# facebookresearch/gtn

Measured on AMD Instinct MI355X. Metric: CTC forward+backward losses/sec (T=1000, C=256), higher is better.
Workload: dtype f32; 1 GPU; BASELINE config C3: compose(ctc_target, emissions)+forwardScore CTC loss fwd+bwd, T=1000, C=256, U=100, batch=512 per GPU; global_batch=512, parallelism=dp1 (utterance sharding, all_gather of losses), rccl_ranks=0

## Files before the change

### gtn_amd/_capi.py

```python
import ctypes as C
import os

c_graph = C.c_void_p
c_graph_p = C.POINTER(C.c_void_p)
c_i32_p = C.POINTER(C.c_int)
c_i64_p = C.POINTER(C.c_int64)
c_u8_p = C.POINTER(C.c_uint8)
c_f32_p = C.POINTER(C.c_float)

GRAD_FN = C.CFUNCTYPE(C.c_int, C.c_void_p, c_graph_p, C.c_int, c_graph)
CTX_FREE = C.CFUNCTYPE(None, C.c_void_p)

OK, INVALID_ARGUMENT, LOGIC_ERROR, RUNTIME_ERROR, OUT_OF_RANGE, DEVICE_ERROR = range(6)

_SIGS = {
    "gtnx_set_device": [C.c_int],
    "gtnx_get_device": [c_i32_p],
    "gtnx_set_stream": [C.c_void_p],
    "gtnx_compose_mode": [C.c_int, C.POINTER(C.c_int)],
    "gtnx_synchronize": [],
    "gtnx_memory_stats": [C.POINTER(C.c_uint64), C.POINTER(C.c_uint64)],
    "gtnx_empty_cache": [],
    "gtnx_reclaim": [],
    "gtnx_graph_create": [C.c_int, c_graph_p],
# ... 94 lines not shown
    "gtnx_batch_align_stats": [c_i64_p, c_i64_p],
    "gtnx_batch_viterbi_decode": [c_graph, c_graph, C.c_void_p, C.c_void_p, C.c_int64, C.c_void_p, C.c_void_p,
                                  C.c_void_p],
    "gtnx_batch_decode_stats": [c_i64_p, c_i64_p],
    "gtnx_batch_full_connect_stats": [c_i64_p, c_i64_p],
    "gtnx_batch_linear_decode": [c_graph, C.c_void_p, C.c_int, C.c_void_p, C.c_int64, C.c_void_p, C.c_void_p,
                                 C.c_void_p, C.c_void_p],
    "gtnx_batch_linear_decode_stats": [c_i64_p, c_i64_p],
    "gtnx_batch_ctc_beam_decode": [c_graph, C.c_void_p, C.c_int, C.c_int, C.c_int, C.c_int, C.c_void_p, C.c_int64,
                                   C.c_void_p, C.c_void_p],
    "gtnx_batch_ctc_beam_stats": [c_i64_p, c_i64_p],
    "gtnx_batch_linear_shape": [c_graph, c_i32_p, c_i32_p],
    "gtnx_batch_edit_distance": [C.c_void_p, C.c_int64, C.c_void_p, C.c_void_p, C.c_int64, C.c_void_p, C.c_int, C.c_int,
                                 C.c_int, C.c_int, C.c_void_p, C.c_void_p],
    "gtnx_batch_edit_distance_stats": [c_i64_p, c_i64_p],
    "gtnx_batch_backward": [c_graph, C.c_int],
    "gtnx_batch_items": [c_graph, C.c_void_p],
    "gtnx_batch_items_device": [c_graph, C.c_void_p],
    "gtnx_batch_grads_bind_device": [c_graph, C.c_void_p, C.c_void_p],
    "gtnx_batch_grads_device": [c_graph, C.c_void_p, C.c_void_p],
    "gtnx_backward": [c_graph, C.c_int],
    "gtnx_backward_with_grad": [c_graph, c_graph, C.c_int],
    "gtnx_backward_n": [c_graph_p, C.c_int, C.c_int],
    "gtnx_equal": [c_graph, c_graph, c_i32_p],
    "gtnx_isomorphic": [c_graph, c_graph, c_i32_p],
    "gtnx_remove": [c_graph, C.c_int, C.c_int, c_graph_p],
    "gtnx_graph_load_buffer": [C.c_void_p, C.c_size_t, c_graph_p],
    "gtnx_parallel_enter": [],
    "gtnx_parallel_leave": [],
    "gtnx_parallel_flush": [],
# ... 55 lines not shown
```

### gtn_amd/criteria/ctc_criterion.h

```cpp
#pragma once

#include <chrono>
#include <cstdint>
#include <stdexcept>
#include <vector>

#include "gtn/gtn.h"

namespace gtn {
namespace criteria {

inline Graph ctcTargetGraph(const std::vector<int>& target, int blank = 0, bool calcGrad = true) {
  const int L = 2 * (int)target.size() + 1;
  std::vector<uint8_t> st(L, 0), ac(L, 0);
  std::vector<int> src, dst, lab;
  src.reserve(3 * L);
  dst.reserve(3 * L);
  lab.reserve(3 * L);
  for (int l = 0; l < L; l++) {
    const int idx = (l - 1) / 2;
    st[l] = l == 0;
    ac[l] = l == L - 1 || l + 2 == L;
    const int label = l % 2 ? target[idx] : blank;
    src.push_back(l), dst.push_back(l), lab.push_back(label);
// ... 18 lines not shown
    int B,
    int T,
    int C,
    int blank,
    void* lossDev,
    void* gradDev,
    bool targetGrad = true,
    CtcStepTimes* times = nullptr,
    Batch* targetsOut = nullptr,
    const int* frames = nullptr) {
  auto now = [] { return std::chrono::steady_clock::now(); };
  auto ms = [](auto a, auto b) { return std::chrono::duration<double, std::milli>(b - a).count(); };
  if (frames)
    for (int b = 0; b < B; ++b)
      if (frames[b] < 1 || frames[b] > T) throw std::invalid_argument("[ctcLossBatch] a frame count outside 1 .. T");
  auto t0 = now();
  Batch ctcs = Batch::ctcTargets(labels, lengths, B, blank, targetGrad);
  auto t1 = now();
  Batch ems = Batch::linear(B, T, C, emissions, gradDev != nullptr, true, frames);
  std::vector<int64_t> off(B);
  for (int b = 0; b < B; ++b) off[b] = (int64_t)b * T * C;
  if (gradDev) ems.bindGrads(gradDev, off.data());
  auto t2 = now();
  Batch comp = batched::intersect(ctcs, ems);
  auto t3 = now();
  Batch score = batched::forwardScore(comp);
  Batch norm = batched::forwardScore(ems);
  Batch losses = batched::subtract(norm, score, lossDev);
  auto t4 = now();
  if (gradDev) batched::backward(losses);
// ... 81 lines not shown
```

### gtn_amd/csrc/band.hip

```cpp
#include <hip/hip_runtime.h>

#include <algorithm>
#include <cstdlib>
#include <stdexcept>
#include <type_traits>

#include "kernels.h"

#ifdef GTNX_BAND_TIMING
__device__ long long g_band_timing[256];
#endif

namespace gtnx {
namespace {

constexpr float NEGF = -1.0e30f;
constexpr float DEADF = -1.0e29f;
constexpr float LOG2E = 1.44269504088896340736f;
constexpr double LN2 = 0.693147180559945309417;
constexpr int BW = 256;
constexpr int WG = 512;
constexpr int WGB = 768;
constexpr int NBE = 5;
constexpr int NBG = 7;
// ... 317 lines not shown
#define GTNX_BAND_PAIR one
#include "band_forward_body.inc"
#undef GTNX_BAND_PAIR
}

__device__ __forceinline__ BandPair band_patched(BandPair P, const BandPatch& pt) {
  if (pt.on) {
    const int b = P.bidx;
    P.delta = pt.delta + b;
    P.delta_norm = pt.delta_norm ? pt.delta_norm + b : nullptr;
    P.rowlse = pt.rowlse ? pt.rowlse + int64_t(b) * pt.M : nullptr;
    P.norm = nullptr;
    P.em_copy = nullptr;
    P.grad_em = pt.grad_em ? pt.grad_em + int64_t(b) * pt.A : nullptr;
    P.grad_fixed = pt.grad_fixed ? pt.grad_fixed + P.goff : nullptr;
  }
  return P;
}
template <int NPL, bool UNIT, bool GRADG, int K, bool VEC, bool BIG>
__global__ __launch_bounds__(WGB, BIG ? 3 : 6) void band_backward_kernel(const BandPair* __restrict__ pairs, int NSmax, BandPatch patch) {
#define GTNX_BAND_PAIR band_patched(pairs[blockIdx.x], patch)
#include "band_backward_body.inc"
#undef GTNX_BAND_PAIR
}
template <int NPL, bool UNIT, bool GRADG, int K, bool VEC, bool BIG>
__global__ __launch_bounds__(WGB, BIG ? 3 : 6) void band_backward_one_kernel(BandPair one, int NSmax) {
#define GTNX_BAND_PAIR one
#include "band_backward_body.inc"
#undef GTNX_BAND_PAIR
}


__global__ __launch_bounds__(512) void ctc_targets_kernel(const CtcTargetArgs* __restrict__ args, int blank) {
  const CtcTargetArgs a = args[blockIdx.x];
  __shared__ __attribute__((aligned(16))) int tl[256 + 4];
  __shared__ __attribute__((aligned(16))) int tk[256 + 4];
  const int N = a.N, U = (N - 1) >> 1, m = threadIdx.x;
  if (m < 260) {
    const int v = m < U ? a.labels[m] : 0x7fffffff;
    tl[m] = v;
    tk[m] = (m > 0 && m < U && v != a.labels[m - 1]) ? 1 : 0;
  }
  __syncthreads();
  if (m >= N) return;
  const bool odd = (m & 1) != 0;
  const int my = odd ? tl[(m - 1) >> 1] : blank;
  const int skip = odd ? tk[(m - 1) >> 1] : 0;
  const int mi = (m - 1) >> 1;
  const int before = odd ? mi : (m >> 1);
  int rank = 0, skips = 0;
  for (int o = 0; o < U; o += 4) {
    const gtnx_i4 l4 = *reinterpret_cast<const gtnx_i4*>(tl + o), k4 = *reinterpret_cast<const gtnx_i4*>(tk + o);
    const int lo[4] = {l4.x, l4.y, l4.z, l4.w}, ko[4] = {k4.x, k4.y, k4.z, k4.w};
#pragma unroll
    for (int k = 0; k < 4; ++k) {
      const bool front = o + k < before;
      rank += (lo[k] < my || (lo[k] == my && front)) ? 1 : 0;
      skips += front ? ko[k] : 0;
    }
  }
  rank += blank < my ? U + 1 : (blank == my ? (m + 1) >> 1 : 0);
  const int base = (m > 0 ? 2 * m - 1 : 0) + skips;
  GTNX_G BandNode* nd = const_cast<GTNX_G BandNode*>(a.nodes);
  nd[m].lab = my;
  nd[m].aid[0] = base;
  nd[m].aid[1] = m > 0 ? base + 1 : -1;
  nd[m].aid[2] = skip ? base + 2 : -1;
  a.nflags[m] = uint8_t((m == 0 ? NF_START : 0) | (m + 2 >= N ? NF_ACCEPT : 0));
  a.snode[rank] = m;
  a.slab[rank] = my;
  if (m == N - 1 && a.n_arcs) a.n_arcs[0] = base + 1 + (m > 0 ? 1 : 0) + skip;
}

__global__ __launch_bounds__(512) void band_viterbi_kernel(const BandDecode* __restrict__ pairs) {
  const BandDecode P = pairs[blockIdx.x];
  const int T = P.T, C = P.C, N = P.N, NS = P.NS;
  extern __shared__ float lds[];
  const float NINF = -__builtin_inff();
  float* a0 = lds;
  float* a1 = lds + 516;
  float* stage = lds + 1032;
  const int m = threadIdx.x;
  const GTNX_G gtnx_i4* nodes = reinterpret_cast<const GTNX_G gtnx_i4*>(P.nodes);
  int lab = 0;
  float wi[3] = {NINF, NINF, NINF};
  bool accept = false, start = false;
// ... 555 lines not shown
  hipLaunchKernelGGL(band_viterbi_kernel, dim3(n), dim3(512), 4 * size_t(1032 + stage_floats) + 64, st, d_pairs);
}

void launch_asg_fal_targets(const AsgFalArgs* d_args, int n, int n_labels, hipStream_t st) {
  if (n > 0) hipLaunchKernelGGL(asg_fal_targets_kernel, dim3(n), dim3(512), 0, st, d_args, n_labels);
}
void launch_asg_fal_scatter(const float* g, const int* maps, const int64_t* tab, int n_seq, int64_t longest, float* trans_grad,
                            hipStream_t st) {
  if (n_seq > 0 && longest > 0)
    hipLaunchKernelGGL(asg_fal_scatter_kernel, dim3(unsigned(std::min<int64_t>((longest + 255) / 256, 64)), unsigned(n_seq)),
                       dim3(256), 0, st, g, maps, tab, trans_grad);
}
void launch_ctc_targets(const CtcTargetArgs* d_args, int n, int blank, hipStream_t st) {
  if (n > 0) hipLaunchKernelGGL(ctc_targets_kernel, dim3(n), dim3(512), 0, st, d_args, blank);
}

}
```

### gtn_amd/csrc/band_backward_body.inc

```
  constexpr int RNk = K >= 4 ? 4 : K;
  constexpr int NP = K / RNk;
  const BandPair P = GTNX_BAND_PAIR;
  const int T = P.T, C = P.C, NS = P.NS;
  extern __shared__ float lds[];
  const BandLds L = band_lds(C, K, NSmax, true);
  float* ering = lds + L.o_ering;
  float* aring = lds + L.o_aring;
  float* oring = lds + L.o_oring;
  int* snode = reinterpret_cast<int*>(lds + L.o_snode);
  const BandMisc M = band_misc<K>(lds, L);
  float* lser = M.lsep;
  const int CS = L.CS;
  const int wv = __builtin_amdgcn_readfirstlane(threadIdx.x >> 6);
  const bool sweeper = wv < 4;
  const int l = threadIdx.x & 63;
  const int nblocks = (T + K - 1) / K;
  const int nticks = nblocks + 5;
  const GTNX_G double* ao = P.aoff;
  const double z2 = uniform(ao[0]);
  const bool dead = !(z2 > double(DEADF));
  const float ds = uniform(P.delta[0]);
  const bool want_em = P.grad_em != nullptr;
  GTNX_TM_INIT(128);
  constexpr bool SPLIT = !BIG && K >= 2 && GTNX_BWD_SPLIT;
  const float dn_k = P.delta_norm ? uniform(P.delta_norm[0]) : 0.0f;
  float* const rnorm_k = lser + NBG * K;
  auto rows_of_k = [&](int c) { return c < nblocks ? min(K, T - c * K) : 0; };
  auto ring_start = [](int c, int M) { return ((c % M) + M) % M; };
  static_assert((NBGE & (NBGE - 1)) == 0, "the emission ring's position is a mask");
  auto ge_of = [](int c) { return int(unsigned(c) & unsigned(NBGE - 1)); };
  auto ring_step = [](int& v, int M) { v = v + 1 == M ? 0 : v + 1; };
  struct RowSumRegs {
    float in[NPL];
    gtnx_f4 hot[NPL];
  };
  auto rowsum_init = [&](RowSumRegs& R) {
#pragma unroll
    for (int q = 0; q < NPL; ++q) {
      const int mb = 256 * q + 4 * l;
      R.in[q] = mb < NSmax ? 1.0f : 0.0f;
// ... 688 lines not shown
```

### gtn_amd/csrc/band_forward_body.inc

```
#ifndef GTNX_FWD_SHIFT_ROWS
#define GTNX_FWD_SHIFT_ROWS 4
#endif
  constexpr int RNk = K >= GTNX_FWD_SHIFT_ROWS ? GTNX_FWD_SHIFT_ROWS : (K >= 4 ? 4 : K);
  constexpr int NP = K / RNk;
  constexpr int D = 8 / K > GTNX_FWD_DEPTH ? 8 / K : GTNX_FWD_DEPTH;
  const BandPair P = GTNX_BAND_PAIR;
  const int T = P.T, C = P.C, NS = P.NS;
  extern __shared__ float lds[];
  const BandLds L = band_lds(C, K, NSmax, false);
  float* ering = lds + L.o_ering;
  const BandMisc M = band_misc<K>(lds, L);
  const int CS = L.CS;
  const int wv = __builtin_amdgcn_readfirstlane(threadIdx.x >> 6);
  const bool sweeper = wv < 4;
  const int l = threadIdx.x & 63;
  const int nblocks = (T + K - 1) / K;
  const int nticks = nblocks + 3;
  GTNX_TM_INIT(0);

  if (sweeper) {
    __builtin_amdgcn_s_setprio(1);
    const int w = wv;
    const int m0 = threadIdx.x * NPL;
    NodeRegs<NPL> g;
// ... 317 lines not shown
    }
    if (hid < 16) M.red[hid] = normacc;
  }
  GTNX_TM_DUMP();
  lds_barrier();
  if (threadIdx.x == 0) {
    double Mx = double(NEGF);
    for (int k = 0; k < 4; ++k)
      if (M.fin[2 * k] > DEADF) Mx = fmax(Mx, M.find[k] + double(M.fin[2 * k]));
    const bool dead = !(Mx > double(DEADF));
    float S = 0.0f;
    for (int k = 0; k < 4; ++k)
      if (M.fin[2 * k] > DEADF) S += M.fin[2 * k + 1] * ex2(float(M.find[k] + double(M.fin[2 * k]) - Mx));
    const double z2 = dead ? double(NEGF) : Mx + double(lg2(S));
    P.aoff[0] = z2;
    P.score[0] = dead ? -__builtin_inff() : float(z2 * LN2);
    if (P.norm) {
      double n2 = 0.0;
      for (int k = 0; k < 16; ++k) n2 += M.red[k];
      P.norm[0] = n2 < double(DEADF) ? -__builtin_inff() : float(n2 * LN2);
    }
  }
```

### gtn_amd/csrc/batch.cpp

```cpp
#include "batch.h"

#include <algorithm>
#include <atomic>
#include <cstdlib>
#include <cstring>
#include <limits>
#include <unordered_map>
#include <unordered_set>

namespace gtnx {

namespace {

std::atomic<uint64_t> g_batch_seq{1};

struct CompMode {
  int old;
  CompMode() : old(compose_mode_hint(2)) {}
  ~CompMode() { compose_mode_hint(old); }
};

BatchP make_batch(Batch::Kind k, int n, bool cg) {
  auto b = std::make_shared<Batch>();
  b->kind = k;
// ... 369 lines not shown
    st[size_t(l)] = l == 0;
    ac[size_t(l)] = l == L - 1 || l + 2 == L;
    const int label = l % 2 ? t[idx] : blank;
    src.push_back(l), dst.push_back(l), lab.push_back(label);
    if (l > 0) src.push_back(l - 1), dst.push_back(l), lab.push_back(label);
    if (l % 2 && l > 1 && label != t[idx - 1]) src.push_back(l - 2), dst.push_back(l), lab.push_back(label);
  }
  Graph g(cg);
  g.add_nodes(L, st.data(), ac.data());
  g.add_arcs(int(src.size()), src.data(), dst.data(), lab.data(), lab.data(), nullptr);
  g.arc_sort(false);
  return g;
}
}

BatchP batch_ctc_targets(const int* labels, const int* lengths, int n, int blank, bool calc_grad) {
  GTNX_HOST_T("batch.ctc_targets");
  if (n < 0) throw_invalid("[gtnx_batch_ctc_targets] negative batch size");
  BatchP b = make_batch(Batch::CTC_TARGETS, n, calc_grad);
  b->blank = blank;
  b->lab_off.resize(size_t(n) + 1);
  b->lab_off[0] = 0;
  for (int i = 0; i < n; ++i) {
    if (lengths[i] < 0) throw_invalid("[gtnx_batch_ctc_targets] negative length");
    b->lab_off[size_t(i) + 1] = b->lab_off[size_t(i)] + lengths[i];
    b->max_nodes = std::max(b->max_nodes, 2 * lengths[i] + 1);
  }
  const size_t total = size_t(b->lab_off[size_t(n)]);
  b->labels.assign(labels, labels + total);
  int mn = blank;
  b->max_label = blank;
  for (size_t i = 0; i < total; ++i) {
    b->max_label = std::max(b->max_label, labels[i]);
    mn = std::min(mn, labels[i]);
  }
  if (mn < 0 || b->max_nodes > band_max_nodes() || n == 0) {
    std::vector<Graph> gs;
    gs.reserve(size_t(n));
    for (int i = 0; i < n; ++i)
      gs.push_back(ctc_target_graph_host(labels + b->lab_off[size_t(i)], lengths[i], blank, calc_grad));
    return batch_from_graphs(std::move(gs));
  }
  Runtime& rt = Runtime::get();
  const size_t lab_bytes = align_up(sizeof(int) * (total ? total : 1), 256);
  const size_t arg_bytes = align_up(sizeof(CtcTargetArgs) * size_t(n), 256);
  size_t bytes = lab_bytes + arg_bytes;
  b->rec_off.resize(size_t(n));
  for (int i = 0; i < n; ++i) {
    const size_t N = size_t(2 * lengths[i] + 1);
    b->rec_off[size_t(i)] = bytes;
    bytes += align_up(sizeof(BandNode) * N, 64) + align_up(N, 64) + 2 * align_up(4 * N, 64) + 64;
  }
  b->rec_mem = rt.alloc(bytes);
  PinnedMemP pin = rt.alloc_pinned(lab_bytes + arg_bytes);
  std::memcpy(pin->ptr, labels, sizeof(int) * total);
  CtcTargetArgs* args = reinterpret_cast<CtcTargetArgs*>(static_cast<char*>(pin->ptr) + lab_bytes);
  for (int i = 0; i < n; ++i) {
    const size_t N = size_t(2 * lengths[i] + 1);
    char* base = b->rec_mem->as<char>(b->rec_off[size_t(i)]);
    CtcTargetArgs& a = args[size_t(i)];
    a.labels = b->rec_mem->as<int>() + b->lab_off[size_t(i)];
    a.nodes = reinterpret_cast<BandNode*>(base);
    base += align_up(sizeof(BandNode) * N, 64);
    a.nflags = reinterpret_cast<uint8_t*>(base);
    base += align_up(N, 64);
    a.snode = reinterpret_cast<int*>(base);
    base += align_up(4 * N, 64);
    a.slab = reinterpret_cast<int*>(base);
    base += align_up(4 * N, 64);
    a.n_arcs = reinterpret_cast<int*>(base);
    a.N = int(N);
    a.pad = 0;
  }
  rt.h2d_pinned(b->rec_mem->ptr, pin->ptr, lab_bytes + arg_bytes);
  launch_ctc_targets(reinterpret_cast<const CtcTargetArgs*>(b->rec_mem->as<char>(lab_bytes)), n, blank, rt.stream());
  return b;
}


BatchP batch_asg_force_align(const int* labels, const int* lengths, int n, Graph& transitions, int n_labels) {
  if (n < 0) throw_invalid("[gtnx_batch_asg_force_align] negative batch size");
  if (transitions.num_nodes() != int64_t(n_labels) + 1 || transitions.num_arcs() != int64_t(n_labels) * (n_labels + 1))
    throw_invalid("[gtnx_batch_asg_force_align] the transitions graph must have the asgTransitions(N) layout");
  BatchP b = make_batch(Batch::CTC_TARGETS, n, transitions.calc_grad());
  b->fal = true;
  b->trans = transitions;
  b->trans_labels = n_labels;
  b->lab_off.resize(size_t(n) + 1);
  b->lab_off[0] = 0;
  int max_u = 0;
  for (int i = 0; i < n; ++i) {
// ... 1423 lines not shown
```

### gtn_amd/csrc/batch.h

```cpp
#pragma once

#include <memory>
#include <vector>

#include "ops.h"

namespace gtnx {

struct Batch;
using BatchP = std::shared_ptr<Batch>;

struct BatchOp {
  uint64_t seq = 0;
  std::vector<BatchP> inputs;
  virtual void backward(Batch& out) = 0;
  virtual ~BatchOp() {}
};

struct Batch {
  enum Kind { GRAPHS, CTC_TARGETS, LINEAR, PRODUCT, SCALAR };
  Kind kind = GRAPHS;
  int n = 0;
  bool calc_grad = false;

// ... 41 lines not shown
  std::shared_ptr<BatchOp> op;
  bool tape_cleared = false;
  DevMemP g_mem;
  float* g_dev = nullptr;
  std::vector<int64_t> g_off;
  DevMemP dest_mem;
  float* dest = nullptr;

  int64_t elem_size(int b) const;
  ~Batch();
};

BatchP batch_from_graphs(std::vector<Graph> gs);
BatchP batch_ctc_targets(const int* labels, const int* lengths, int n, int blank, bool calc_grad);
BatchP batch_asg_force_align(const int* labels, const int* lengths, int n, Graph& transitions, int n_labels);
BatchP batch_linear(int n, int M, int C, bool calc_grad, const void* dev, bool borrow, const int* rows = nullptr);
BatchP batch_compose(const BatchP& a, const BatchP& b, bool intersect);
BatchP batch_shortest_distance(const BatchP& x, bool tropical);
void batch_full_connect_stats(int64_t* fast, int64_t* fallback);
BatchP batch_viterbi_path(const BatchP& x);
void batch_viterbi_align(const BatchP& x, const int* frames, int* labels_dev, int64_t row_stride, int* tokens_dev,
                         float* scores_dev);
void batch_align_stats(int64_t* fast, int64_t* fallback);
void batch_viterbi_decode(const BatchP& ems, Graph& transitions, const int* frames, int* labels_dev, int64_t row_stride,
                          float* scores_dev, int* collapsed_dev, int* lengths_dev);
void batch_decode_stats(int64_t* fast, int64_t* fallback);
void batch_linear_decode(const BatchP& ems, const int* frames, int blank, int* labels_dev, int64_t row_stride,
                         float* scores_dev, int* collapsed_dev, int* starts_dev, int* lengths_dev);
void batch_linear_decode_stats(int64_t* fast, int64_t* fallback);
void batch_ctc_beam_decode(const BatchP& ems, const int* frames, int blank, int beam, int topn, int nbest,
// ... 21 lines not shown
```

### gtn_amd/csrc/capi.cpp

```cpp
#include <atomic>
#include <chrono>
#include <condition_variable>
#include <cstdlib>
#include <cstring>
#include <mutex>
#include <string>
#include <vector>

#include "batch.h"
#include "ops.h"
#include "ops_internal.h"
#include "region.h"

#define GTNX_API extern "C" __attribute__((visibility("default")))

using namespace gtnx;

namespace {
thread_local std::string g_err;

gtnx_status_t fail(gtnx_status_t s, const std::string& m) {
  g_err = m;
  return s;
}
// ... 730 lines not shown

namespace {
inline BatchP& BH(gtnx_batch_t h) {
  if (!h) throw_invalid("null batch handle");
  return *reinterpret_cast<BatchP*>(h);
}
inline gtnx_batch_t HB(BatchP b) { return reinterpret_cast<gtnx_batch_t>(new BatchP(std::move(b))); }
}
GTNX_API gtnx_status_t gtnx_batch_from_graphs(const gtnx_graph_t* g, int n, gtnx_batch_t* out) {
  return guard([&] { *out = HB(batch_from_graphs(vec(g, n, true))); });
}
GTNX_API gtnx_status_t gtnx_batch_ctc_targets(const int* labels, const int* lengths, int n, int blank, int cg,
                                              gtnx_batch_t* out) {
  return guard([&] { *out = HB(batch_ctc_targets(labels, lengths, n, blank, cg != 0)); });
}
GTNX_API gtnx_status_t gtnx_batch_asg_force_align(const int* labels, const int* lengths, int n, gtnx_graph_t transitions,
                                                  int n_labels, gtnx_batch_t* out) {
  return guard([&] { *out = HB(batch_asg_force_align(labels, lengths, n, G(transitions), n_labels)); });
}
GTNX_API gtnx_status_t gtnx_batch_linear(int n, int M, int N, int cg, const void* dev, int borrow, gtnx_batch_t* out) {
  return guard([&] { *out = HB(batch_linear(n, M, N, cg != 0, dev, borrow != 0)); });
}
GTNX_API gtnx_status_t gtnx_batch_linear_rows(int n, int M, int N, const int* rows, int cg, const void* dev, int borrow,
                                             gtnx_batch_t* out) {
  return guard([&] { *out = HB(batch_linear(n, M, N, cg != 0, dev, borrow != 0, rows)); });
}
GTNX_API gtnx_status_t gtnx_batch_destroy(gtnx_batch_t b) {
  return guard([&] {
    auto* p = reinterpret_cast<BatchP*>(b);
    if (!p) return;
// ... 210 lines not shown
```

### gtn_amd/csrc/kernels.h

```cpp
#pragma once

#include <hip/hip_runtime.h>

#include <cstdint>

#include <atomic>
#include <cstdint>
struct gtnx_first_on_device {
  std::atomic<uint64_t>& done;
  uint64_t bit;
  bool first;
  explicit gtnx_first_on_device(std::atomic<uint64_t>& d) : done(d) {
    int dev = 0;
    (void)hipGetDevice(&dev);
    bit = uint64_t(1) << (dev & 63);
    first = !(done.load(std::memory_order_acquire) & bit);
  }
  gtnx_first_on_device(const gtnx_first_on_device&) = delete;
  ~gtnx_first_on_device() {
    if (first) done.fetch_or(bit, std::memory_order_acq_rel);
  }
  explicit operator bool() const { return first; }
};

// ... 340 lines not shown
  GTNX_G float* alpha;
  GTNX_G double* aoff;
  GTNX_G float* score;
  GTNX_G float* norm;
  GTNX_G float* rowlse;
  const GTNX_G float* delta;
  const GTNX_G float* delta_norm;
  GTNX_G float* grad_em;
  GTNX_G float* grad_fixed;
  int N, T, C, NS;
  int hot;
  int lgrn;
  int n_lab;
  int bidx;
  int64_t goff;
};
struct BandPatch {
  int on;
  int M;
  const GTNX_G float* delta;
  const GTNX_G float* delta_norm;
  GTNX_G float* rowlse;
  GTNX_G float* grad_em;
  GTNX_G float* grad_fixed;
  int64_t A;
};
struct BandDecode {
  const GTNX_G BandNode* nodes;
  const GTNX_G uint8_t* nflags;
  const GTNX_G float* w;
  const GTNX_G float* em;
  GTNX_G uint8_t* bp;
  GTNX_G int* pnode;
  GTNX_G int* path_arc;
  GTNX_G int* path_lab;
  GTNX_G float* path_w;
  GTNX_G int* path_len;
  GTNX_G float* score;
  GTNX_G int* tie;
  const GTNX_G int* rank_in;
// ... 77 lines not shown
void launch_remove_walk(const RemoveArgs& a, bool emit, hipStream_t st);
size_t scan_temp_bytes(int n);
void launch_exclusive_scan(const int* in, int* out, int n, void* temp, size_t temp_bytes, hipStream_t st);
void launch_rational_load(const void* rows, const float* w, const uint8_t* flags, const RationalOut& out, void* temp,
                          hipStream_t st);
struct CtcTargetArgs {
  const GTNX_G int* labels;
  GTNX_G BandNode* nodes;
  GTNX_G uint8_t* nflags;
  GTNX_G int* snode;
  GTNX_G int* slab;
  GTNX_G int* n_arcs;
  int N, pad;
};
void launch_ctc_targets(const CtcTargetArgs* d_args, int n, int blank, hipStream_t st);
struct AsgFalArgs {
  const GTNX_G int* labels;
  const GTNX_G float* trans_w;
  GTNX_G BandNode* nodes;
  GTNX_G uint8_t* nflags;
  GTNX_G int* snode;
  GTNX_G int* slab;
  GTNX_G float* w;
  GTNX_G int* arc_map;
  int U, pad;
};
void launch_asg_fal_targets(const AsgFalArgs* d_args, int n, int n_labels, hipStream_t st);
void launch_asg_fal_scatter(const float* g, const int* maps, const int64_t* tab , int n_seq, int64_t longest,
                            float* trans_grad, hipStream_t st);
int band_max_nodes();
// ... 147 lines not shown
```

### include/gtn/batch.h

```cpp
#pragma once
#include <cstdint>
#include <utility>
#include <vector>

#include "gtn/functions.h"

namespace gtn {

class Batch {
 public:
  Batch() = default;
  explicit Batch(const std::vector<Graph>& graphs) {
    auto h = detail::handles(graphs);
    detail::check(gtnx_batch_from_graphs(h.data(), static_cast<int>(h.size()), &h_));
  }
  Batch(const Batch&) = delete;
  Batch& operator=(const Batch&) = delete;
  Batch(Batch&& o) noexcept : h_(o.h_) { o.h_ = nullptr; }
  Batch& operator=(Batch&& o) noexcept {
    if (this != &o) {
      reset();
      h_ = o.h_;
      o.h_ = nullptr;
    }
// ... 5 lines not shown
    std::vector<int> flat, len;
    len.reserve(targets.size());
    size_t total = 0;
    for (auto& t : targets) total += t.size();
    flat.reserve(total);
    for (auto& t : targets) {
      flat.insert(flat.end(), t.begin(), t.end());
      len.push_back(static_cast<int>(t.size()));
    }
    return ctcTargets(flat.data(), len.data(), static_cast<int>(targets.size()), blank, calcGrad);
  }
  static Batch ctcTargets(const int* labels, const int* lengths, int n, int blank = 0, bool calcGrad = true) {
    Batch b;
    detail::check(gtnx_batch_ctc_targets(labels, lengths, n, blank, calcGrad, &b.h_));
    return b;
  }
  static Batch asgForceAlign(const int* labels, const int* lengths, int n, const Graph& transitions, int numLabels) {
    Batch b;
    detail::check(gtnx_batch_asg_force_align(labels, lengths, n, transitions.handle(), numLabels, &b.h_));
    return b;
  }
  static Batch linear(int n, int M, int N, const void* deviceWeights, bool calcGrad = true, bool borrow = false,
                      const int* rows = nullptr) {
    Batch b;
    if (rows)
      detail::check(gtnx_batch_linear_rows(n, M, N, rows, calcGrad, deviceWeights, borrow, &b.h_));
    else
      detail::check(gtnx_batch_linear(n, M, N, calcGrad, deviceWeights, borrow, &b.h_));
    return b;
  }
// ... 98 lines not shown
```

### include/gtn_amd.h

```cpp
#ifndef GTN_AMD_H
#define GTN_AMD_H

#include <stddef.h>
#include <stdint.h>

#ifdef __cplusplus
extern "C" {
#endif

typedef int gtnx_status_t;
#define GTNX_OK 0
#define GTNX_INVALID_ARGUMENT 1
#define GTNX_LOGIC_ERROR 2
#define GTNX_RUNTIME_ERROR 3
#define GTNX_OUT_OF_RANGE 4
#define GTNX_DEVICE_ERROR 5

typedef struct gtnx_graph_s* gtnx_graph_t;

#define GTNX_EPSILON (-1)

const char* gtnx_last_error(void);
const char* gtnx_version(void);
const char* gtnx_backend(void);
// ... 95 lines not shown
gtnx_status_t gtnx_items_n(const gtnx_graph_t* g, int n, float* out);
gtnx_status_t gtnx_items_device_n(const gtnx_graph_t* g, int n, void* device_out);
gtnx_status_t gtnx_grads_device_n(const gtnx_graph_t* g, int n, void* device_out, const int64_t* offsets);
gtnx_status_t gtnx_grads_bind_device_n(const gtnx_graph_t* g, int n, void* device_out, const int64_t* offsets);

gtnx_status_t gtnx_clone(gtnx_graph_t g, int projection , gtnx_graph_t* out);
gtnx_status_t gtnx_concat(const gtnx_graph_t* g, int n, gtnx_graph_t* out);
gtnx_status_t gtnx_closure(gtnx_graph_t g, gtnx_graph_t* out);
gtnx_status_t gtnx_union(const gtnx_graph_t* g, int n, gtnx_graph_t* out);
gtnx_status_t gtnx_remove(gtnx_graph_t g, int ilabel, int olabel, gtnx_graph_t* out);

typedef struct gtnx_batch_s* gtnx_batch_t;
gtnx_status_t gtnx_batch_from_graphs(const gtnx_graph_t* g, int n, gtnx_batch_t* out);
gtnx_status_t gtnx_batch_ctc_targets(const int* labels, const int* lengths, int n, int blank, int calc_grad,
                                     gtnx_batch_t* out);
gtnx_status_t gtnx_batch_asg_force_align(const int* labels, const int* lengths, int n, gtnx_graph_t transitions,
                                         int n_labels, gtnx_batch_t* out);
gtnx_status_t gtnx_batch_linear(int n, int M, int N, int calc_grad, const void* device_weights, int borrow,
                                gtnx_batch_t* out);
gtnx_status_t gtnx_batch_linear_rows(int n, int M, int N, const int* rows, int calc_grad, const void* device_weights,
                                     int borrow, gtnx_batch_t* out);
gtnx_status_t gtnx_batch_destroy(gtnx_batch_t b);
gtnx_status_t gtnx_batch_size(gtnx_batch_t b, int* out);
gtnx_status_t gtnx_batch_get(gtnx_batch_t b, int i, gtnx_graph_t* out);
gtnx_status_t gtnx_batch_negate(gtnx_batch_t a, gtnx_batch_t* out);
gtnx_status_t gtnx_batch_add(gtnx_batch_t a, gtnx_batch_t b, gtnx_batch_t* out);
gtnx_status_t gtnx_batch_subtract(gtnx_batch_t a, gtnx_batch_t b, gtnx_batch_t* out);
gtnx_status_t gtnx_batch_subtract_into(gtnx_batch_t a, gtnx_batch_t b, void* items_device, gtnx_batch_t* out);
gtnx_status_t gtnx_batch_compose(gtnx_batch_t a, gtnx_batch_t b, gtnx_batch_t* out);
gtnx_status_t gtnx_batch_intersect(gtnx_batch_t a, gtnx_batch_t b, gtnx_batch_t* out);
// ... 61 lines not shown
```

Baseline: 935,700 losses/s.

## Add fused CTC loss path building targets, band forward and backward in few launches

Adds a fused CTC loss route that builds the target records, the band pair table and the arena on the host in one pass. One head kernel both emits the CTC target records and copies the pair table from pinned memory, then runs band forward (writing loss = norm - score directly) and band backward with constant seed deltas. This skips the separate linear batch, intersect, the two forwardScore calls, the subtract and the generic backward dispatch. It costs a large new code path that declines to the old route on unusual shapes, and it reads pinned host memory directly from a kernel.

```diff
diff --git a/gtn_amd/_capi.py b/gtn_amd/_capi.py
--- a/gtn_amd/_capi.py
+++ b/gtn_amd/_capi.py
@@ -132,6 +132,9 @@
     "gtnx_batch_edit_distance": [C.c_void_p, C.c_int64, C.c_void_p, C.c_void_p, C.c_int64, C.c_void_p, C.c_int, C.c_int,
                                  C.c_int, C.c_int, C.c_void_p, C.c_void_p],
     "gtnx_batch_edit_distance_stats": [c_i64_p, c_i64_p],
+    "gtnx_batch_ctc_loss_fused": [C.c_void_p, C.c_void_p, C.c_void_p, C.c_int, C.c_int, C.c_int, C.c_int, C.c_void_p,
+                                  C.c_void_p, C.c_void_p, C.c_int, C.c_void_p, C.POINTER(C.c_int), C.POINTER(C.c_double)],
+    "gtnx_batch_ctc_fused_stats": [c_i64_p, c_i64_p],
     "gtnx_batch_backward": [c_graph, C.c_int],
     "gtnx_batch_items": [c_graph, C.c_void_p],
     "gtnx_batch_items_device": [c_graph, C.c_void_p],
diff --git a/gtn_amd/criteria/ctc_criterion.h b/gtn_amd/criteria/ctc_criterion.h
--- a/gtn_amd/criteria/ctc_criterion.h
+++ b/gtn_amd/criteria/ctc_criterion.h
@@ -56,6 +56,16 @@
   if (frames)
     for (int b = 0; b < B; ++b)
       if (frames[b] < 1 || frames[b] > T) throw std::invalid_argument("[ctcLossBatch] a frame count outside 1 .. T");
+  if (emissions && lengths && lossDev) {
+    Batch fused;
+    double hms[3] = {0, 0, 0};
+    if (Batch::ctcLossFused(emissions, labels, lengths, B, T, C, blank, frames, lossDev, gradDev, targetGrad, &fused, hms) ==
+        GTNX_CTC_FUSED_TAKEN) {
+      if (times) *times = {hms[0], 0, 0, hms[1], hms[2]};
+      if (targetsOut) *targetsOut = std::move(fused);
+      return;
+    }
+  }
   auto t0 = now();
   Batch ctcs = Batch::ctcTargets(labels, lengths, B, blank, targetGrad);
   auto t1 = now();
diff --git a/gtn_amd/csrc/band.hip b/gtn_amd/csrc/band.hip
--- a/gtn_amd/csrc/band.hip
+++ b/gtn_amd/csrc/band.hip
@@ -355,32 +355,44 @@
     P.em_copy = nullptr;
     P.grad_em = pt.grad_em ? pt.grad_em + int64_t(b) * pt.A : nullptr;
     P.grad_fixed = pt.grad_fixed ? pt.grad_fixed + P.goff : nullptr;
+    if (pt.seed) {
+      P.delta = P.score;
+      P.delta_norm = P.score;
+    }
   }
   return P;
 }
 template <int NPL, bool UNIT, bool GRADG, int K, bool VEC, bool BIG>
 __global__ __launch_bounds__(WGB, BIG ? 3 : 6) void band_backward_kernel(const BandPair* __restrict__ pairs, int NSmax, BandPatch patch) {
 #define GTNX_BAND_PAIR band_patched(pairs[blockIdx.x], patch)
+#define GTNX_BAND_DELTA(P) (patch.seed ? patch.seed_delta : uniform((P).delta[0]))
+#define GTNX_BAND_DELTA_NORM(P) (patch.seed ? patch.seed_delta_norm : ((P).delta_norm ? uniform((P).delta_norm[0]) : 0.0f))
 #include "band_backward_body.inc"
+#undef GTNX_BAND_DELTA_NORM
+#undef GTNX_BAND_DELTA
 #undef GTNX_BAND_PAIR
 }
 template <int NPL, bool UNIT, bool GRADG, int K, bool VEC, bool BIG>
 __global__ __launch_bounds__(WGB, BIG ? 3 : 6) void band_backward_one_kernel(BandPair one, int NSmax) {
 #define GTNX_BAND_PAIR one
+#define GTNX_BAND_DELTA(P) uniform((P).delta[0])
+#define GTNX_BAND_DELTA_NORM(P) ((P).delta_norm ? uniform((P).delta_norm[0]) : 0.0f)
 #include "band_backward_body.inc"
+#undef GTNX_BAND_DELTA_NORM
+#undef GTNX_BAND_DELTA
 #undef GTNX_BAND_PAIR
 }
 
 
-__global__ __launch_bounds__(512) void ctc_targets_kernel(const CtcTargetArgs* __restrict__ args, int blank) {
-  const CtcTargetArgs a = args[blockIdx.x];
+__device__ __forceinline__ void ctc_target_records(const CtcTargetArgs& a, const GTNX_G int* src, bool keep, int blank) {
   __shared__ __attribute__((aligned(16))) int tl[256 + 4];
   __shared__ __attribute__((aligned(16))) int tk[256 + 4];
   const int N = a.N, U = (N - 1) >> 1, m = threadIdx.x;
   if (m < 260) {
-    const int v = m < U ? a.labels[m] : 0x7fffffff;
+    const int v = m < U ? src[m] : 0x7fffffff;
     tl[m] = v;
-    tk[m] = (m > 0 && m < U && v != a.labels[m - 1]) ? 1 : 0;
+    tk[m] = (m > 0 && m < U && v != src[m - 1]) ? 1 : 0;
+    if (keep && m < U) const_cast<GTNX_G int*>(a.labels)[m] = v;
   }
   __syncthreads();
   if (m >= N) return;
@@ -411,6 +423,22 @@
   a.snode[rank] = m;
   a.slab[rank] = my;
   if (m == N - 1 && a.n_arcs) a.n_arcs[0] = base + 1 + (m > 0 ? 1 : 0) + skip;
+}
+__global__ __launch_bounds__(512) void ctc_targets_kernel(const CtcTargetArgs* __restrict__ args, int blank) {
+  const CtcTargetArgs a = args[blockIdx.x];
+  ctc_target_records(a, a.labels, false, blank);
+}
+__global__ __launch_bounds__(512) void ctc_head_kernel(const CtcTargetArgs* __restrict__ h_args, int n, int blank,
+                                                       const int* __restrict__ h_labels, const int* d_labels,
+                                                       const gtnx_i4* __restrict__ h_table, gtnx_i4* d_table, int table_vecs) {
+  if (int(blockIdx.x) >= n) {
+    const int stride = int(gridDim.x - n) * 512;
+    for (int i = int(blockIdx.x - n) * 512 + int(threadIdx.x); i < table_vecs; i += stride) d_table[i] = h_table[i];
+    return;
+  }
+  const CtcTargetArgs a = h_args[blockIdx.x];
+  const size_t off = (reinterpret_cast<uintptr_t>(a.labels) - reinterpret_cast<uintptr_t>(d_labels)) / sizeof(int);
+  ctc_target_records(a, (const GTNX_G int*)(h_labels + off), true, blank);
 }
 
 __global__ __launch_bounds__(512) void band_viterbi_kernel(const BandDecode* __restrict__ pairs) {
@@ -996,5 +1024,14 @@
 void launch_ctc_targets(const CtcTargetArgs* d_args, int n, int blank, hipStream_t st) {
   if (n > 0) hipLaunchKernelGGL(ctc_targets_kernel, dim3(n), dim3(512), 0, st, d_args, blank);
 }
-
-}
+void launch_ctc_head(const CtcTargetArgs* h_args, int n, int blank, const int* h_labels, int* d_labels, const void* h_table,
+                     void* d_table, size_t table_bytes, hipStream_t st) {
+  if (n <= 0) return;
+  if (table_bytes % 16 != 0 || table_bytes / 16 > size_t(1) << 30) throw std::logic_error("band.hip: the head's table is copied in 16-byte words");
+  const int vecs = int(table_bytes / 16);
+  const int copiers = std::min((vecs + 511) / 512, 64);
+  hipLaunchKernelGGL(ctc_head_kernel, dim3(n + copiers), dim3(512), 0, st, h_args, n, blank, h_labels, d_labels,
+                     static_cast<const gtnx_i4*>(h_table), static_cast<gtnx_i4*>(d_table), vecs);
+}
+
+}
diff --git a/gtn_amd/csrc/band_backward_body.inc b/gtn_amd/csrc/band_backward_body.inc
--- a/gtn_amd/csrc/band_backward_body.inc
+++ b/gtn_amd/csrc/band_backward_body.inc
@@ -19,11 +19,11 @@
   const GTNX_G double* ao = P.aoff;
   const double z2 = uniform(ao[0]);
   const bool dead = !(z2 > double(DEADF));
-  const float ds = uniform(P.delta[0]);
+  const float ds = GTNX_BAND_DELTA(P);
   const bool want_em = P.grad_em != nullptr;
   GTNX_TM_INIT(128);
   constexpr bool SPLIT = !BIG && K >= 2 && GTNX_BWD_SPLIT;
-  const float dn_k = P.delta_norm ? uniform(P.delta_norm[0]) : 0.0f;
+  const float dn_k = GTNX_BAND_DELTA_NORM(P);
   float* const rnorm_k = lser + NBG * K;
   auto rows_of_k = [&](int c) { return c < nblocks ? min(K, T - c * K) : 0; };
   auto ring_start = [](int c, int M) { return ((c % M) + M) % M; };
diff --git a/gtn_amd/csrc/band_forward_body.inc b/gtn_amd/csrc/band_forward_body.inc
--- a/gtn_amd/csrc/band_forward_body.inc
+++ b/gtn_amd/csrc/band_forward_body.inc
@@ -355,10 +355,14 @@
       if (M.fin[2 * k] > DEADF) S += M.fin[2 * k + 1] * ex2(float(M.find[k] + double(M.fin[2 * k]) - Mx));
     const double z2 = dead ? double(NEGF) : Mx + double(lg2(S));
     P.aoff[0] = z2;
-    P.score[0] = dead ? -__builtin_inff() : float(z2 * LN2);
+    const float sc = dead ? -__builtin_inff() : float(z2 * LN2);
+    P.score[0] = sc;
     if (P.norm) {
       double n2 = 0.0;
       for (int k = 0; k < 16; ++k) n2 += M.red[k];
-      P.norm[0] = n2 < double(DEADF) ? -__builtin_inff() : float(n2 * LN2);
+      const float nrm = n2 < double(DEADF) ? -__builtin_inff() : float(n2 * LN2);
+      P.norm[0] = nrm;
+      GTNX_G float* const loss = (GTNX_BAND_PAIR).loss;
+      if (loss) loss[0] = nrm - sc;
     }
   }
diff --git a/gtn_amd/csrc/batch.cpp b/gtn_amd/csrc/batch.cpp
--- a/gtn_amd/csrc/batch.cpp
+++ b/gtn_amd/csrc/batch.cpp
@@ -2,6 +2,7 @@
 
 #include <algorithm>
 #include <atomic>
+#include <chrono>
 #include <cstdlib>
 #include <cstring>
 #include <limits>
@@ -407,8 +408,8 @@
 }
 }
 
-BatchP batch_ctc_targets(const int* labels, const int* lengths, int n, int blank, bool calc_grad) {
-  GTNX_HOST_T("batch.ctc_targets");
+namespace {
+BatchP ctc_targets_record(const int* labels, const int* lengths, int n, int blank, bool calc_grad, bool* band) {
   if (n < 0) throw_invalid("[gtnx_batch_ctc_targets] negative batch size");
   BatchP b = make_batch(Batch::CTC_TARGETS, n, calc_grad);
   b->blank = blank;
@@ -427,32 +428,33 @@
     b->max_label = std::max(b->max_label, labels[i]);
     mn = std::min(mn, labels[i]);
   }
-  if (mn < 0 || b->max_nodes > band_max_nodes() || n == 0) {
-    std::vector<Graph> gs;
-    gs.reserve(size_t(n));
-    for (int i = 0; i < n; ++i)
-      gs.push_back(ctc_target_graph_host(labels + b->lab_off[size_t(i)], lengths[i], blank, calc_grad));
-    return batch_from_graphs(std::move(gs));
-  }
-  Runtime& rt = Runtime::get();
-  const size_t lab_bytes = align_up(sizeof(int) * (total ? total : 1), 256);
-  const size_t arg_bytes = align_up(sizeof(CtcTargetArgs) * size_t(n), 256);
-  size_t bytes = lab_bytes + arg_bytes;
-  b->rec_off.resize(size_t(n));
+  *band = !(mn < 0 || b->max_nodes > band_max_nodes() || n == 0);
+  return b;
+}
+struct CtcRecLayout {
+  size_t lab_bytes, arg_bytes, bytes;
+};
+CtcRecLayout ctc_targets_layout(Batch& b, const int* lengths) {
+  const int n = b.n;
+  const size_t total = size_t(b.lab_off[size_t(n)]);
+  CtcRecLayout L;
+  L.lab_bytes = align_up(sizeof(int) * (total ? total : 1), 256);
+  L.arg_bytes = align_up(sizeof(CtcTargetArgs) * size_t(n), 256);
+  L.bytes = L.lab_bytes + L.arg_bytes;
+  b.rec_off.resize(size_t(n));
   for (int i = 0; i < n; ++i) {
     const size_t N = size_t(2 * lengths[i] + 1);
-    b->rec_off[size_t(i)] = bytes;
-    bytes += align_up(sizeof(BandNode) * N, 64) + align_up(N, 64) + 2 * align_up(4 * N, 64) + 64;
-  }
-  b->rec_mem = rt.alloc(bytes);
-  PinnedMemP pin = rt.alloc_pinned(lab_bytes + arg_bytes);
-  std::memcpy(pin->ptr, labels, sizeof(int) * total);
-  CtcTargetArgs* args = reinterpret_cast<CtcTargetArgs*>(static_cast<char*>(pin->ptr) + lab_bytes);
-  for (int i = 0; i < n; ++i) {
+    b.rec_off[size_t(i)] = L.bytes;
+    L.bytes += align_up(sizeof(BandNode) * N, 64) + align_up(N, 64) + 2 * align_up(4 * N, 64) + 64;
+  }
+  return L;
+}
+void ctc_targets_args(Batch& b, const int* lengths, CtcTargetArgs* args) {
+  for (int i = 0; i < b.n; ++i) {
     const size_t N = size_t(2 * lengths[i] + 1);
-    char* base = b->rec_mem->as<char>(b->rec_off[size_t(i)]);
+    char* base = b.rec_mem->as<char>(b.rec_off[size_t(i)]);
     CtcTargetArgs& a = args[size_t(i)];
-    a.labels = b->rec_mem->as<int>() + b->lab_off[size_t(i)];
+    a.labels = b.rec_mem->as<int>() + b.lab_off[size_t(i)];
     a.nodes = reinterpret_cast<BandNode*>(base);
     base += align_up(sizeof(BandNode) * N, 64);
     a.nflags = reinterpret_cast<uint8_t*>(base);
@@ -465,9 +467,199 @@
     a.N = int(N);
     a.pad = 0;
   }
-  rt.h2d_pinned(b->rec_mem->ptr, pin->ptr, lab_bytes + arg_bytes);
-  launch_ctc_targets(reinterpret_cast<const CtcTargetArgs*>(b->rec_mem->as<char>(lab_bytes)), n, blank, rt.stream());
+}
+}
+
+BatchP batch_ctc_targets(const int* labels, const int* lengths, int n, int blank, bool calc_grad) {
+  GTNX_HOST_T("batch.ctc_targets");
+  bool band = false;
+  BatchP b = ctc_targets_record(labels, lengths, n, blank, calc_grad, &band);
+  if (!band) {
+    std::vector<Graph> gs;
+    gs.reserve(size_t(n));
+    for (int i = 0; i < n; ++i)
+      gs.push_back(ctc_target_graph_host(labels + b->lab_off[size_t(i)], lengths[i], blank, calc_grad));
+    return batch_from_graphs(std::move(gs));
+  }
+  Runtime& rt = Runtime::get();
+  const size_t total = size_t(b->lab_off[size_t(n)]);
+  const CtcRecLayout L = ctc_targets_layout(*b, lengths);
+  b->rec_mem = rt.alloc(L.bytes);
+  PinnedMemP pin = rt.alloc_pinned(L.lab_bytes + L.arg_bytes);
+  std::memcpy(pin->ptr, labels, sizeof(int) * total);
+  ctc_targets_args(*b, lengths, reinterpret_cast<CtcTargetArgs*>(static_cast<char*>(pin->ptr) + L.lab_bytes));
+  rt.h2d_pinned(b->rec_mem->ptr, pin->ptr, L.lab_bytes + L.arg_bytes);
+  launch_ctc_targets(reinterpret_cast<const CtcTargetArgs*>(b->rec_mem->as<char>(L.lab_bytes)), n, blank, rt.stream());
   return b;
+}
+
+namespace {
+std::atomic<int64_t> g_ctc_fused{0}, g_ctc_declined{0};
+int ctc_declined(int why) {
+  g_ctc_declined.fetch_add(1);
+  return why;
+}
+}
+void batch_ctc_fused_stats(int64_t* fused, int64_t* declined) {
+  if (fused) *fused = g_ctc_fused.load();
+  if (declined) *declined = g_ctc_declined.load();
+}
+int batch_ctc_loss_fused(const void* emissions, const int* labels, const int* lengths, int n, int T, int C, int blank,
+                         const int* frames, void* loss_dev, void* grad_dev, bool target_grad, BatchP* targets_out,
+                         double* host_ms) {
+  GTNX_HOST_T("batch.ctc_loss_fused");
+  if (!emissions || !lengths || !loss_dev) throw_invalid("[gtnx_batch_ctc_loss_fused] null emissions, lengths or loss pointer");
+  if (targets_out) targets_out->reset();
+  if (host_ms) host_ms[0] = host_ms[1] = host_ms[2] = 0.0;
+  const char* sw = std::getenv("GTNX_CTC_FUSED");
+  if (sw && sw[0] == '0') return ctc_declined(CTC_FUSED_OFF);
+  if (std::getenv("GTNX_H2D_KERNEL_BYTES") || std::getenv("GTNX_NO_BAND_PATCH") || std::getenv("GTNX_LAZY_COMPOSE"))
+    return ctc_declined(CTC_FUSED_SWITCH);
+  if (n <= 0 || T < 1 || T > (1 << 20) || C < band_min_labels() || C > band_max_labels()) return ctc_declined(CTC_FUSED_SHAPE);
+  int64_t total_labels = 0;
+  for (int i = 0; i < n; ++i) {
+    if (lengths[i] < 0) return ctc_declined(CTC_FUSED_SHAPE);
+    total_labels += lengths[i];
+  }
+  if (total_labels > 0 && !labels) throw_invalid("[gtnx_batch_ctc_loss_fused] null labels");
+  bool band = false;
+  BatchP fx = ctc_targets_record(labels, lengths, n, blank, target_grad, &band);
+  if (!band || fx->max_label >= C) return ctc_declined(CTC_FUSED_SHAPE);
+  const int npl = band_npl(2 * lengths[0] + 1);
+  for (int i = 1; i < n; ++i)
+    if (band_npl(2 * lengths[i] + 1) != npl) return ctc_declined(CTC_FUSED_SHAPE);
+  int64_t pad_rows = 0;
+  if (frames)
+    for (int i = 0; i < n; ++i) {
+      if (frames[i] < 1 || frames[i] > T) throw_invalid("[gtnx_batch_linear_rows] a row count outside 1 .. M");
+      pad_rows += T - frames[i];
+    }
+  Runtime& rt = Runtime::get();
+  if (!ptr_local_to(emissions, rt.device()) || !ptr_local_to(loss_dev, rt.device()) ||
+      (grad_dev && !ptr_local_to(grad_dev, rt.device())))
+    return ctc_declined(CTC_FUSED_FOREIGN);
+  auto now = [] { return std::chrono::steady_clock::now(); };
+  auto ms = [](auto a, auto b) { return std::chrono::duration<double, std::milli>(b - a).count(); };
+  const auto t0 = now();
+  const size_t total = size_t(total_labels);
+  const CtcRecLayout L = ctc_targets_layout(*fx, lengths);
+  fx->rec_mem = rt.alloc(L.bytes);
+  size_t abytes_total = align_up(4 * size_t(n), 256);
+  const size_t o_norm = abytes_total;
+  abytes_total = align_up(abytes_total + 4 * size_t(n), 256);
+  const size_t o_lse = abytes_total;
+  abytes_total = align_up(abytes_total + 4 * size_t(n) * size_t(T), 256);
+  std::vector<size_t> oo, ao;
+  oo.resize(size_t(n));
+  ao.resize(size_t(n));
+  for (int b = 0; b < n; ++b) {
+    const int N = 2 * lengths[b] + 1;
+    oo[size_t(b)] = abytes_total;
+    abytes_total = align_up(abytes_total + 8 * (4 * size_t(T) + 16), 256);
+    ao[size_t(b)] = abytes_total;
+    abytes_total = align_up(abytes_total + 4 * size_t(T + 1) * size_t(band_row_stride(N, band_npl(N))), 256);
+  }
+  DevMemP arena = rt.alloc(abytes_total);
+  const bool backward = grad_dev != nullptr;
+  if (backward && target_grad) alloc_grad(*fx, false);
+  const size_t pair_bytes = align_up(sizeof(BandPair) * size_t(n), 256);
+  const size_t rows_bytes = align_up(sizeof(int) * size_t(n), 256);
+  const size_t padt_bytes = pad_rows > 0 && backward ? align_up(rows_bytes + 8 * (size_t(n) + 1), 256) : 0;
+  const size_t table_bytes = pair_bytes + padt_bytes;
+  PinnedMemP pin = rt.alloc_pinned(L.lab_bytes + L.arg_bytes + table_bytes);
+  DevMemP table = rt.alloc(table_bytes);
+  char* const hp = static_cast<char*>(pin->ptr);
+  if (total) std::memcpy(hp, labels, sizeof(int) * total);
+  ctc_targets_args(*fx, lengths, reinterpret_cast<CtcTargetArgs*>(hp + L.lab_bytes));
+  BandPair* pairs = reinterpret_cast<BandPair*>(hp + L.lab_bytes + L.arg_bytes);
+  std::memset(pairs, 0, table_bytes);
+  const float* em = static_cast<const float*>(emissions);
+  const bool vec = C % 4 == 0 && (reinterpret_cast<uintptr_t>(em) & 15) == 0;
+  const int lgrn = band_forward_lgrn(C);
+  int max_ns = 0;
+  int64_t goff_run = 0;
+  double fbytes = 0, bbytes = 0;
+  for (int b = 0; b < n; ++b) {
+    BandPair& p = pairs[b];
+    const int U = lengths[b];
+    const size_t N = size_t(2 * U + 1);
+    char* base = fx->rec_mem->as<char>(fx->rec_off[size_t(b)]);
+    p.nodes = reinterpret_cast<BandNode*>(base);
+    base += align_up(sizeof(BandNode) * N, 64);
+    p.nflags = reinterpret_cast<uint8_t*>(base);
+    base += align_up(N, 64);
+    p.snode = reinterpret_cast<int*>(base);
+    base += align_up(4 * N, 64);
+    p.slab = reinterpret_cast<int*>(base);
+    p.n_lab = int(N);
+    p.em = em + size_t(b) * size_t(T) * size_t(C);
+    p.N = int(N);
+    p.T = frames ? frames[b] : T;
+    p.C = C;
+    p.NS = band_row_stride(p.N, band_npl(p.N));
+    p.alpha = arena->as<float>(ao[size_t(b)]);
+    p.aoff = arena->as<double>(oo[size_t(b)]);
+    p.score = arena->as<float>(4 * size_t(b));
+    p.norm = arena->as<float>(o_norm + 4 * size_t(b));
+    p.rowlse = arena->as<float>(o_lse + 4 * size_t(b) * size_t(T));
+    p.loss = static_cast<float*>(loss_dev) + b;
+    p.hot = U + 1 >= 8 ? blank : -1;
+    p.lgrn = lgrn;
+    p.bidx = b;
+    p.goff = goff_run;
+    goff_run += fx->elem_size(b);
+    max_ns = std::max(max_ns, p.NS);
+    fbytes += 4.0 * p.T * C + 4.0 * double(p.T + 1) * p.NS;
+    bbytes += 4.0 * p.T * C * 2 + 4.0 * double(p.T + 1) * p.NS + (fx->g_dev ? 4.0 * double(fx->elem_size(b)) : 0.0);
+  }
+  Batch ems_pad;
+  if (padt_bytes) {
+    char* const ht = hp + L.lab_bytes + L.arg_bytes + pair_bytes;
+    std::memcpy(ht, frames, sizeof(int) * size_t(n));
+    int64_t* prefix = reinterpret_cast<int64_t*>(ht + rows_bytes);
+    prefix[0] = 0;
+    for (int i = 0; i < n; ++i) prefix[i + 1] = prefix[i] + int64_t(T - frames[i]) * C;
+    ems_pad.kind = Batch::LINEAR;
+    ems_pad.n = n;
+    ems_pad.M = T;
+    ems_pad.C = C;
+    ems_pad.rows.assign(frames, frames + n);
+    ems_pad.pad_floats = pad_rows * C;
+    ems_pad.pad_mem = std::make_shared<DevMem>();
+    ems_pad.pad_mem->ptr = table->as<char>(pair_bytes);
+    ems_pad.pad_mem->bytes = padt_bytes;
+    ems_pad.pad_mem->borrowed = true;
+    ems_pad.pad_mem->keep = table;
+  }
+  launch_ctc_head(reinterpret_cast<const CtcTargetArgs*>(hp + L.lab_bytes), n, blank, reinterpret_cast<const int*>(hp),
+                  fx->rec_mem->as<int>(), pairs, table->ptr, table_bytes, rt.stream());
+  const auto t1 = now();
+  {
+    GTNX_PROF("band_forward_score", fbytes);
+    launch_band_forward(table->as<BandPair>(), n, npl, C, max_ns, true, vec, rt.stream());
+  }
+  const auto t2 = now();
+  if (backward) {
+    if (padt_bytes) pad_fill(ems_pad, static_cast<float*>(grad_dev));
+    BandPatch pt{};
+    pt.on = 1;
+    pt.M = T;
+    pt.rowlse = arena->as<float>(o_lse);
+    pt.grad_em = static_cast<float*>(grad_dev);
+    pt.grad_fixed = fx->g_dev;
+    pt.A = int64_t(T) * C;
+    pt.seed = 1;
+    pt.seed_delta = -1.0f;
+    pt.seed_delta_norm = 1.0f;
+    GTNX_PROF("band_forward_score_grad", bbytes);
+    launch_band_backward(table->as<BandPair>(), n, npl, C, max_ns, true, fx->g_dev != nullptr, vec, rt.stream(),
+                         nullptr, &pt);
+  }
+  const auto t3 = now();
+  if (host_ms) host_ms[0] = ms(t0, t1), host_ms[1] = ms(t1, t2), host_ms[2] = ms(t2, t3);
+  g_ctc_fused.fetch_add(1);
+  if (targets_out) *targets_out = fx;
+  return CTC_FUSED_TAKEN;
 }
 
 
diff --git a/gtn_amd/csrc/batch.h b/gtn_amd/csrc/batch.h
--- a/gtn_amd/csrc/batch.h
+++ b/gtn_amd/csrc/batch.h
@@ -79,6 +79,17 @@
 BatchP batch_from_graphs(std::vector<Graph> gs);
 BatchP batch_ctc_targets(const int* labels, const int* lengths, int n, int blank, bool calc_grad);
 BatchP batch_asg_force_align(const int* labels, const int* lengths, int n, Graph& transitions, int n_labels);
+enum {
+  CTC_FUSED_TAKEN = 1,
+  CTC_FUSED_OFF = 0,
+  CTC_FUSED_SWITCH = -1,
+  CTC_FUSED_SHAPE = -2,
+  CTC_FUSED_FOREIGN = -3,
+};
+int batch_ctc_loss_fused(const void* emissions, const int* labels, const int* lengths, int n, int T, int C, int blank,
+                         const int* frames, void* loss_dev, void* grad_dev, bool target_grad, BatchP* targets_out,
+                         double* host_ms);
+void batch_ctc_fused_stats(int64_t* fused, int64_t* declined);
 BatchP batch_linear(int n, int M, int C, bool calc_grad, const void* dev, bool borrow, const int* rows = nullptr);
 BatchP batch_compose(const BatchP& a, const BatchP& b, bool intersect);
 BatchP batch_shortest_distance(const BatchP& x, bool tropical);
diff --git a/gtn_amd/csrc/capi.cpp b/gtn_amd/csrc/capi.cpp
--- a/gtn_amd/csrc/capi.cpp
+++ b/gtn_amd/csrc/capi.cpp
@@ -768,6 +768,22 @@
                                               gtnx_batch_t* out) {
   return guard([&] { *out = HB(batch_ctc_targets(labels, lengths, n, blank, cg != 0)); });
 }
+GTNX_API gtnx_status_t gtnx_batch_ctc_loss_fused(const void* emissions, const int* labels, const int* lengths, int n, int T,
+                                                 int C, int blank, const int* frames, void* loss_device, void* grad_device,
+                                                 int target_grad, gtnx_batch_t* targets_out, int* route, double* host_ms) {
+  return guard([&] {
+    if (!route) throw_invalid("[gtnx_batch_ctc_loss_fused] null route pointer");
+    *route = GTNX_CTC_FUSED_OFF;
+    if (targets_out) *targets_out = nullptr;
+    BatchP fx;
+    *route = batch_ctc_loss_fused(emissions, labels, lengths, n, T, C, blank, frames, loss_device, grad_device, target_grad != 0,
+                                  &fx, host_ms);
+    if (targets_out && fx) *targets_out = HB(std::move(fx));
+  });
+}
+GTNX_API gtnx_status_t gtnx_batch_ctc_fused_stats(int64_t* fused, int64_t* declined) {
+  return guard([&] { batch_ctc_fused_stats(fused, declined); });
+}
 GTNX_API gtnx_status_t gtnx_batch_asg_force_align(const int* labels, const int* lengths, int n, gtnx_graph_t transitions,
                                                   int n_labels, gtnx_batch_t* out) {
   return guard([&] { *out = HB(batch_asg_force_align(labels, lengths, n, G(transitions), n_labels)); });
diff --git a/gtn_amd/csrc/kernels.h b/gtn_amd/csrc/kernels.h
--- a/gtn_amd/csrc/kernels.h
+++ b/gtn_amd/csrc/kernels.h
@@ -378,6 +378,7 @@
   int n_lab;
   int bidx;
   int64_t goff;
+  GTNX_G float* loss;
 };
 struct BandPatch {
   int on;
@@ -388,6 +389,9 @@
   GTNX_G float* grad_em;
   GTNX_G float* grad_fixed;
   int64_t A;
+  int seed;
+  float seed_delta, seed_delta_norm;
+  int pad;
 };
 struct BandDecode {
   const GTNX_G BandNode* nodes;
@@ -495,6 +499,8 @@
   int N, pad;
 };
 void launch_ctc_targets(const CtcTargetArgs* d_args, int n, int blank, hipStream_t st);
+void launch_ctc_head(const CtcTargetArgs* h_args, int n, int blank, const int* h_labels, int* d_labels, const void* h_table,
+                     void* d_table, size_t table_bytes, hipStream_t st);
 struct AsgFalArgs {
   const GTNX_G int* labels;
   const GTNX_G float* trans_w;
diff --git a/include/gtn/batch.h b/include/gtn/batch.h
--- a/include/gtn/batch.h
+++ b/include/gtn/batch.h
@@ -43,6 +43,17 @@
     Batch b;
     detail::check(gtnx_batch_ctc_targets(labels, lengths, n, blank, calcGrad, &b.h_));
     return b;
+  }
+  static int ctcLossFused(const void* emissions, const int* labels, const int* lengths, int n, int T, int C, int blank,
+                          const int* frames, void* lossDevice, void* gradDevice, bool targetGrad, Batch* targets,
+                          double* hostMs = nullptr) {
+    int route = GTNX_CTC_FUSED_OFF;
+    gtnx_batch_t h = nullptr;
+    detail::check(gtnx_batch_ctc_loss_fused(emissions, labels, lengths, n, T, C, blank, frames, lossDevice, gradDevice,
+                                            targetGrad, &h, &route, hostMs));
+    if (targets) *targets = fromHandle(h);
+    else if (h) gtnx_batch_destroy(h);
+    return route;
   }
   static Batch asgForceAlign(const int* labels, const int* lengths, int n, const Graph& transitions, int numLabels) {
     Batch b;
diff --git a/include/gtn_amd.h b/include/gtn_amd.h
--- a/include/gtn_amd.h
+++ b/include/gtn_amd.h
@@ -133,6 +133,15 @@
 gtnx_status_t gtnx_batch_from_graphs(const gtnx_graph_t* g, int n, gtnx_batch_t* out);
 gtnx_status_t gtnx_batch_ctc_targets(const int* labels, const int* lengths, int n, int blank, int calc_grad,
                                      gtnx_batch_t* out);
+#define GTNX_CTC_FUSED_TAKEN 1
+#define GTNX_CTC_FUSED_OFF 0
+#define GTNX_CTC_FUSED_SWITCH (-1)
+#define GTNX_CTC_FUSED_SHAPE (-2)
+#define GTNX_CTC_FUSED_FOREIGN (-3)
+gtnx_status_t gtnx_batch_ctc_loss_fused(const void* emissions, const int* labels, const int* lengths, int n, int T, int C,
+                                        int blank, const int* frames, void* loss_device, void* grad_device, int target_grad,
+                                        gtnx_batch_t* targets_out, int* route, double* host_ms);
+gtnx_status_t gtnx_batch_ctc_fused_stats(int64_t* fused, int64_t* declined);
 gtnx_status_t gtnx_batch_asg_force_align(const int* labels, const int* lengths, int n, gtnx_graph_t transitions,
                                          int n_labels, gtnx_batch_t* out);
 gtnx_status_t gtnx_batch_linear(int n, int M, int N, int calc_grad, const void* device_weights, int borrow,
```

Result: faster. 952,000 losses/s (median of 6 runs) (+1.7%).
